# Project-SEA-Stack/HydroChrono

Measured on AMD Instinct MI355X. Metric: hydro-force evals/sec (all bodies), higher is better.
Workload: dtype f64

## Files before the change

hydrochrono_amd/capi.py:

```python
import ctypes as C
import os

_PKG = os.path.dirname(os.path.abspath(__file__))
LIB_PATH = os.path.join(_PKG, "lib", "libhydrochrono_amd.so")
TUNING_LIB_PATH = os.path.join(_PKG, "lib", "libhydrochrono_amd_tuning.so")

HC_OK, HC_ERR_RUNTIME, HC_ERR_OUT_OF_RANGE, HC_ERR_INVALID, HC_ERR_DEVICE, HC_ERR_UNSUPPORTED = range(6)

c_double_p = C.POINTER(C.c_double)
c_int_p = C.POINTER(C.c_int)


class IrregularWaveParams(C.Structure):
    _fields_ = [("num_bodies", C.c_int), ("simulation_dt", C.c_double), ("simulation_duration", C.c_double),
                ("ramp_duration", C.c_double), ("wave_height", C.c_double), ("wave_period", C.c_double),
                ("frequency_min", C.c_double), ("frequency_max", C.c_double), ("nfrequencies", C.c_double),
                ("peak_enhancement_factor", C.c_double), ("is_normalized", C.c_int), ("seed", C.c_int)]


class TaperedDirectOptions(C.Structure):
    _fields_ = [("smoothing", C.c_int), ("window_length", C.c_int), ("rirf_end_time", C.c_double),
                ("taper_start_percent", C.c_double), ("taper_end_percent", C.c_double),
                ("taper_final_amplitude", C.c_double), ("export_plot_csv", C.c_int)]

# ... 12 lines not shown


class MorisonMember(C.Structure):
    _fields_ = [("r0", C.c_double * 3), ("r1", C.c_double * 3), ("d0", C.c_double), ("d1", C.c_double), ("cd", C.c_double),
                ("cm", C.c_double), ("n_seg", C.c_int)]


class SurfacePanel(C.Structure):
    _fields_ = [("c", C.c_double * 3), ("s", C.c_double * 3)]


class RadiationMode(C.Structure):
    _fields_ = [("row", C.c_int), ("col", C.c_int), ("lambda_re", C.c_double), ("lambda_im", C.c_double),
                ("rho_re", C.c_double), ("rho_im", C.c_double)]


class ProfileStats(C.Structure):
    _fields_ = [("hydrostatics_seconds", C.c_double), ("radiation_seconds", C.c_double), ("waves_seconds", C.c_double),
                ("hydrostatics_calls", C.c_int), ("radiation_calls", C.c_int), ("waves_calls", C.c_int),
                ("conv_kernel_seconds", C.c_double), ("conv_kernel_launches", C.c_longlong),
                ("conv_kernel_bytes", C.c_double), ("block_kernel_seconds", C.c_double),
                ("block_kernel_launches", C.c_longlong), ("block_kernel_bytes", C.c_double),
                ("block_kernel_bytes_once", C.c_double),
                ("step_kernel_seconds", C.c_double), ("step_kernel_launches", C.c_longlong),
                ("scatter_kernel_seconds", C.c_double), ("scatter_kernel_launches", C.c_longlong),
                ("direct_dispatches", C.c_longlong), ("hip_launches", C.c_longlong), ("history_rewinds", C.c_longlong),
                ("mini_pass_seconds", C.c_double), ("mini_pass_launches", C.c_longlong), ("queue_parkings", C.c_longlong),
                ("ahead_pass_slices", C.c_longlong), ("ahead_blocks", C.c_longlong),
                ("pass_lane_launches", C.c_longlong),
                ("multi_doorbell_offset_last", C.c_double), ("multi_doorbell_offset_sum", C.c_double), ("multi_calls", C.c_longlong),
                ("slot_state_steps", C.c_longlong), ("wide_fused_steps", C.c_longlong),
                ("schedule_blocks_ahead", C.c_longlong), ("schedule_blocks_at_start", C.c_longlong), ("ring_grows_for_pass", C.c_longlong),
                ("hot_steps", C.c_longlong), ("tail_launches", C.c_longlong), ("tail_seconds", C.c_double),
                ("tail_bytes", C.c_double), ("tail_blocks", C.c_longlong)]


class InitStats(C.Structure):
    _fields_ = [("h5_read_seconds", C.c_double), ("h5_read_bytes", C.c_double), ("rirf_h2d_seconds", C.c_double), ("rirf_h2d_bytes", C.c_double),
                ("rirf_relayout_seconds", C.c_double), ("rirf_relayout_bytes", C.c_double), ("finalize_seconds", C.c_double),
                ("direct_setup_seconds", C.c_double), ("wave_resample_seconds", C.c_double), ("wave_spectrum_seconds", C.c_double),
                ("wave_eta_seconds", C.c_double), ("wave_eta_samples", C.c_longlong), ("wave_eta_components", C.c_longlong),
                ("wave_eta_mode", C.c_int), ("pad_", C.c_int), ("wave_upload_seconds", C.c_double), ("wave_upload_bytes", C.c_double),
                ("wave_total_seconds", C.c_double), ("taper_seconds", C.c_double), ("taper_bytes", C.c_double),
                ("synth_seconds", C.c_double), ("synth_bytes", C.c_double)]


SIGNATURES = {
    "hc_version": (C.c_char_p, []),
    "hc_device_count": (C.c_int, []),
    "hc_device_local_cpus": (C.c_int, [C.c_int, C.c_char_p, C.c_size_t]),
    "hc_bind_thread_to_device": (C.c_int, [C.c_int]),
    "hc_create": (C.c_int, [C.c_int, C.c_int, C.POINTER(C.c_void_p)]),
    "hc_create_sharded": (C.c_int, [C.c_int, C.c_int, C.c_int, C.c_int, C.POINTER(C.c_void_p)]),
    "hc_destroy": (None, [C.c_void_p]),
    "hc_last_error": (C.c_char_p, [C.c_void_p]),
    "hc_set_simulation_parameters": (C.c_int, [C.c_void_p, C.c_double, C.c_double, C.c_double]),
    "hc_set_body_properties": (C.c_int, [C.c_void_p, C.c_int, C.c_double, c_double_p, c_double_p]),
    "hc_set_hydrostatic_stiffness": (C.c_int, [C.c_void_p, C.c_int, c_double_p]),
    "hc_set_added_mass_inf": (C.c_int, [C.c_void_p, C.c_int, c_double_p]),
    "hc_set_rirf": (C.c_int, [C.c_void_p, C.c_int, c_double_p, C.c_int, c_double_p]),
    "hc_set_excitation_rao": (C.c_int, [C.c_void_p, C.c_int, c_double_p, C.c_int, c_double_p, c_double_p]),
    "hc_set_excitation_irf": (C.c_int, [C.c_void_p, C.c_int, c_double_p, C.c_int, c_double_p]),
    "hc_load_bemio_h5": (C.c_int, [C.c_void_p, C.c_char_p]),
    "hc_finalize": (C.c_int, [C.c_void_p]),
    "hc_set_gravity": (C.c_int, [C.c_void_p, c_double_p]),
    "hc_set_wave_none": (C.c_int, [C.c_void_p, C.c_int]),
    "hc_set_wave_regular": (C.c_int, [C.c_void_p, C.c_int, C.c_double, C.c_double]),
# ... 212 lines not shown
```

hydrochrono_amd/csrc/hc_context.hpp:

```cpp
#pragma once
#include <hip/hip_runtime.h>

#include <chrono>
#include <cmath>
#include <deque>
#include <stdexcept>
#include <string>
#include <vector>

#include "../../include/hydrochrono_amd.h"
#include "hc_direct.hpp"
#include "hc_kernels.hpp"
#include "hc_plan.hpp"

namespace hc {

struct Error : std::runtime_error {
    int status;
    Error(int st, const std::string& what) : std::runtime_error(what), status(st) {}
};

#define HC_HIP(expr)                                                                                          \
    do {                                                                                                      \
        hipError_t _e = (expr);                                                                               \
// ... 205 lines not shown
    int first_body = 0, off = 0, L = 0;
    double tau_front = 0.0, tau_back = 0.0;
};

enum WaveKind { kWaveNone = 0, kWaveRegular = 1, kWaveIrregular = 2, kWaveSpectral = 3 };

enum EventKind { kEvConvPlain = 0, kEvPass = 1, kEvStep = 2, kEvScatter = 3, kEvConvExc = 4, kEvMiniPass = 5, kEvTail = 6 };
struct EventPair {
    hipEvent_t a = nullptr, b = nullptr;
    int kind = 0;
    double waves_share = 0.0;
};

}

struct hc_ctx {
    int N = 0, b0 = 0, b1 = 0, nloc = 0, D = 0, Dloc = 0, device = 0;
    hipStream_t stream = nullptr;
    hipStream_t stream_am = nullptr;
    hipEvent_t ev_fin = nullptr, ev_bg = nullptr;
    bool bg_pending = false;
    hipStream_t last_stream = nullptr;
    bool have_last_stream   = false;
    hc::DirectQueue* dq = nullptr;
    bool direct_ready   = false;
    std::string direct_why;
    std::string direct_how = "direct AQL dispatch";
    int path            = 0;
    hc::DirectKernel dk_finalize_slot;
    hc::DirectKernel dk_step_hot[2];
    bool step_hot = false;
    int step_halves = 1;
    bool slot_state = false;
    hc::DirectKernel dk_finalize, dk_scatter, dk_reduce, dk_block16, dk_block32, dk_block64, dk_mini16, dk_mini32, dk_narrow, dk_wide, dk_added_mass, dk_step, dk_near;
    hc::StepTail tail;
    int pending_step  = 0;
    double pending_t  = 0.0;
    int pending_am    = 0;
    bool lost         = false;
    int arm_mode = 1;
    bool arm_after_step = false, arm_after_am = false;
    std::chrono::steady_clock::time_point t_step_end{}, t_am_end{};
    bool have_t_step_end = false, have_t_am_end = false;
    int busy_caller_steps   = 0;
    std::string err;

    bool have_sim = false;
    double rho = 0, g = 0, depth = 0;
    double gsys[3] = {0.0, 0.0, -9.81};
    std::vector<hc::BodyHost> bodies;

    int S = 0;
    std::vector<double> tau, width;
    hc::DeviceBuffer<double> dK, dKproc, d_tau, d_width, d_stage;
    int ntiles = 0, Dpad = 0, ngp = 0, mt = 1, ngroups = 0;
    int conv_mode = 0;
    bool proc_ready = false;
    hc_tapered_direct_options taper{};
    std::string diagnostics_dir;
    bool finalized = false;

    std::deque<double> times;
    std::deque<double> retired;
    int head = -1, Hcap = 0, HcapT = 0;
    hc::DeviceBuffer<double> d_ring_t, d_ring_v, d_ring_vT;
    long long rewinds = 0;
    bool have_prev = false, have_prev_device = false;
// ... 146 lines not shown
```

hydrochrono_amd/csrc/hc_internal.hpp:

```cpp
#pragma once
#include <dlfcn.h>
#include <fcntl.h>
#include <unistd.h>
#include <xmmintrin.h>

#include <algorithm>
#include <chrono>
#include <cmath>
#include <cstdint>
#include <cstdio>
#include <cstdlib>
#include <cstring>
#include <fstream>
#include <limits>
#include <memory>
#include <string>
#include <vector>

#include "hc_context.hpp"
#include "hc_history.hpp"
#include "hc_host_math.hpp"

namespace hc {
void eta_synthesis_fft(const std::vector<double>& t, const std::vector<double>& amp, const std::vector<double>& omega,
// ... 112 lines not shown
    return RaoBracket{k0, k0 + 1, idx_des - std::floor(idx_des)};
}
inline void rao_bracket_check(const RaoBracket& br, int nw) {
    if (br.k0 < 0 || br.k0 + 1 >= nw) throw Error(HC_ERR_OUT_OF_RANGE, "regular wave frequency outside the BEM frequency list");
}
void apply_wave_directions(hc_ctx* c, const std::vector<double>& theta, bool commit, bool force);

struct StepFlags {
    bool hs = true, rad = true, waves = true;
    bool scratch_out = false;
};
struct HostState {
    const double *pos, *rpy, *linvel, *angvel;
    double canary;
};
void enqueue_step(hc_ctx* c, double t, const double* d_state, double* d_user_out, hipStream_t stream, StepFlags f,
                  unsigned long long* host_tagged = nullptr, unsigned long long seq = 0, bool defer_tail = false, const HostState* host_state = nullptr);
void enqueue_tail(hc_ctx* c);

bool wave_window_ok(const hc_ctx* c, double t);
int live_samples(const hc_ctx* c, double t_query);
double* rows_P(hc_ctx* c, bool next);
double* rows_E(hc_ctx* c, bool next);

struct StepViews {
    hc::Panel kex;
    hc::EtaTable ex;
};
StepViews make_views(const hc_ctx* c);
struct PassSetup {
    hc::BlockArgs b;
    bool exc_block = false;
    double rad_once = 0.0, exc_once = 0.0, bytes_steps = 0.0;
};
PassSetup make_pass(hc_ctx* c, bool with_exc, bool next_block, int head_lags = 0);
void issue_pass_chunks(hc_ctx* c, const PassSetup& ps, int first, int last, bool with_items, hipStream_t stream, bool direct, int lane = 0);
struct TailRows {
    const double* tail[hc::kTailLevelsMax] = {nullptr, nullptr, nullptr};
    int j0[hc::kTailLevelsMax]             = {0, 0, 0};
};
void issue_pass_reduce(hc_ctx* c, const PassSetup& ps, double* P, double* E, hipStream_t stream, bool direct, int lane = 0, const TailRows* tail = nullptr);
void launch_pass(hc_ctx* c, hipStream_t stream, bool with_exc, bool direct = false, bool spec_goes_on = false);
void spec_drop(hc_ctx* c, bool k_changed);
void spec_build_khat(hc_ctx* c, hc_ctx::SpectralLevel& lev);
void launch_mini_pass(hc_ctx* c, int i0, hipStream_t stream, bool direct, int next_kw = 0, int lane = 0);
void ahead_drop(hc_ctx* c);
void ahead_issue_slice(hc_ctx* c, hipStream_t stream, bool direct);
void ahead_begin(hc_ctx* c, hipStream_t stream, bool with_exc, bool direct);
bool ahead_expected(const hc_ctx* c, unsigned long long ended_serial);
bool ahead_adoptable(const hc_ctx* c, unsigned long long ended_serial);
bool pass_lane_ready(hc_ctx* c);
void pass_lane_drain(hc_ctx* c);

}
}
```

hydrochrono_amd/csrc/hc_kernels.hip:

```cpp
#include "hc_kernels.hpp"

#include <algorithm>
#include <cstdint>
#include <cstdlib>

namespace hc {

static constexpr int kConvThreads = 256;
static constexpr int kWave        = 64;

typedef double dvec2 __attribute__((ext_vector_type(2)));
typedef double dvec2u __attribute__((ext_vector_type(2), aligned(8)));
typedef double dvec4 __attribute__((ext_vector_type(4)));

__host__ __device__ inline size_t panel_offset(int ngp, int row, int f) {
    const int rt = row >> 4, ri = row & 15, gp = f >> 3, j = (f >> 2) & 1, kk = f & 3;
    return ((static_cast<size_t>(rt) * ngp + gp) * 64 + (kk * 16 + ri)) * 2 + j;
}

__global__ void __launch_bounds__(256) relayout_rirf_kernel(const double* __restrict__ Kb, double* __restrict__ K, int ngp, int D, int S,
                                                             int row0, double scale) {
    const size_t F   = (size_t)S * D;
    const size_t gid = (size_t)blockIdx.x * blockDim.x + threadIdx.x;
    if (gid >= 6 * F) return;
// ... 716 lines not shown
                ++s_c;
            } while (cb_c >= D);
            load_weights();
        }
    };

    const int nfrag = (gp1 - gp0 - wave + 3) / 4;
#pragma unroll
    for (int r = 0; r < R; ++r) issue(r);
    for (int i = 0; i < nfrag; i += R) {
#pragma unroll
        for (int r = 0; r < R; ++r) {
            consume(r);
            issue(r);
        }
    }

#pragma unroll
    for (int tb = 0; tb < NB; ++tb) {
        __syncthreads();
#pragma unroll
        for (int m = 0; m < MT; ++m)
#pragma unroll
            for (int r = 0; r < 4; ++r) red[((size_t)wave * MT + m) * 256 + (kk + 4 * r) * 16 + jstep] = acc[tb][m][r];
        __syncthreads();
        for (int idx = tid; idx < MT * 256; idx += kConvThreads) {
            const int m = idx >> 8, el = idx & 255, row = el >> 4, j = el & 15;
            const double v = ((red[(0 * MT + m) * 256 + el] + red[(1 * MT + m) * 256 + el]) + red[(2 * MT + m) * 256 + el]) + red[(3 * MT + m) * 256 + el];
            a.partials[((size_t)chunk * L + 16 * tb + j) * a.Dpad + (grp * MT + m) * 16 + row] = v;
        }
    }
}

template <int MT, int R, int NB, int WPS = (NB == 1 ? 2 : 1)>
__global__ void __launch_bounds__(kConvThreads, WPS) conv_block_kernel(BlockArgs a) {
    extern __shared__ __align__(16) unsigned char smem_raw[];
    double* front = reinterpret_cast<double*>(smem_raw);
    const int nt  = a.max_steps_per_chunk * 16 * NB;
    double* t_wo  = front + a.lds_front_doubles;
    double* t_wn  = t_wo + nt;
    int* t_oo     = reinterpret_cast<int*>(t_wn + nt);
    int* t_on     = t_oo + nt;

    const int r     = (int)blockIdx.x % (8 * a.ngroups);
    const int chunk = a.chunk_first + ((int)blockIdx.x / (8 * a.ngroups)) * 8 + (r & 7);
    const int grp   = r >> 3;
    if (chunk >= (a.chunk_last > 0 ? a.chunk_last : a.nchunks)) return;

    if constexpr (NB > 2) {
        block_rad_stream_uni<MT, R, NB>(a, chunk, grp, front, t_wo, t_wn, t_oo, t_on);
    } else {
        if ((a.hist.D & 7) == 0 && (size_t)a.hist.D * a.hist.HcapT < ((size_t)1 << 28)) block_rad_stream_uni<MT, R, NB>(a, chunk, grp, front, t_wo, t_wn, t_oo, t_on);
        else block_rad_stream<MT, (NB > 1) ? 2 : R, NB, false>(a, chunk, grp, front, t_wo, t_wn, t_oo, t_on);
    }
    const int RG      = a.ngroups;
    const int n_items = a.nchunks_ex * NB * RG;
    if (n_items > 0) {
        __shared__ int s_item;
        for (;;) {
            __syncthreads();
            if (threadIdx.x == 0) s_item = atomicAdd(a.item_counter, 1);
            __syncthreads();
            const int it = s_item;
            if (it >= n_items) break;
            const int e = it / (NB * RG), rem = it - e * (NB * RG), tb = rem / RG, rg = rem - tb * RG;
            block_exc_work<MT>(a, rg, e, 16 * tb, front);
        }
    }
}

template <class KernelT>
static void allow_dynamic_lds(KernelT kernel, size_t smem, size_t& granted) {
    if (smem > 64 * 1024 && smem > granted) {
        (void)hipFuncSetAttribute(reinterpret_cast<const void*>(kernel), hipFuncAttributeMaxDynamicSharedMemorySize, (int)smem);
        granted = smem;
    }
}

template <int MT, int R>
static void launch_conv_block_mt(const BlockArgs& b, int nblocks, size_t smem, hipStream_t stream) {
    static size_t granted16 = 0, granted32 = 0;
    if (b.depth == 32) {
        allow_dynamic_lds(conv_block_kernel<MT, R + 1, 2>, smem, granted32);
        hipLaunchKernelGGL((conv_block_kernel<MT, R + 1, 2>), dim3(nblocks), dim3(kConvThreads), smem, stream, b);
    } else {
        allow_dynamic_lds(conv_block_kernel<MT, R, 1>, smem, granted16);
        hipLaunchKernelGGL((conv_block_kernel<MT, R, 1>), dim3(nblocks), dim3(kConvThreads), smem, stream, b);
    }
}

#ifdef HC_TUNING
static void launch_conv_block64(const BlockArgs& b, int nblocks, size_t smem, hipStream_t stream) {
    static size_t granted = 0;
    allow_dynamic_lds(conv_block_kernel<kBlock64MT, 4, 4, 1>, smem, granted);
    hipLaunchKernelGGL((conv_block_kernel<kBlock64MT, 4, 4, 1>), dim3(nblocks), dim3(kConvThreads), smem, stream, b);
}
#endif

BlockLaunch block_launch_config(const BlockArgs& a, int mt, BlockArgs* b) {
    BlockLaunch l;
    const int nlaunch = (a.chunk_last > 0 ? a.chunk_last : a.nchunks) - a.chunk_first;
// ... 1 lines not shown
    *b        = a;
    b->lds_front_doubles = max(4 * kUWave, 4 * mt * 256);
    l.smem    = (size_t)b->lds_front_doubles * sizeof(double) + (size_t)max(1, a.max_steps_per_chunk) * b->depth * 24;
#ifdef HC_TUNING
    if (a.depth == 64) {
        l.MT  = kBlock64MT;
        l.NB  = 4;
        l.R   = 4;
        l.WPS = 1;
        return l;
    }
#endif
    l.MT  = (mt == 6 || mt == 4 || mt == 2) ? mt : 1;
    const int R16 = l.MT == 6 ? 3 : 4;
    l.NB  = a.depth == 32 ? 2 : 1;
    l.R   = a.depth == 32 ? R16 + 1 : R16;
    l.WPS = l.NB == 1 ? 2 : 1;
    return l;
}

void launch_conv_block(const BlockArgs& a, int mt, hipStream_t stream) {
    BlockArgs b;
    const BlockLaunch l = block_launch_config(a, mt, &b);
    const int nblocks   = l.nblocks;
    const size_t smem   = l.smem;
    if (nblocks <= 0) return;
#ifdef HC_TUNING
    if (b.depth == 64) { launch_conv_block64(b, nblocks, smem, stream); return; }
#endif
    if (mt == 6) launch_conv_block_mt<6, 3>(b, nblocks, smem, stream);
    else if (mt == 4) launch_conv_block_mt<4, 4>(b, nblocks, smem, stream);
    else if (mt == 2) launch_conv_block_mt<2, 4>(b, nblocks, smem, stream);
    else launch_conv_block_mt<1, 4>(b, nblocks, smem, stream);
}

__device__ __forceinline__ double lane16_sum(double v) {
#pragma unroll
    for (int off = 8; off >= 1; off >>= 1) v += __shfl_xor(v, off, 16);
    return v;
}

__global__ void __launch_bounds__(256) reduce_block_kernel(ReduceArgs a) {
    if (blockIdx.x == 0 && threadIdx.x == 0) *a.item_counter = 0;
    const double* __restrict__ partials = a.partials;
    const int sub = threadIdx.x & 15;
    const int n   = a.depth * a.Dpad;
    int out       = blockIdx.x * 16 + (threadIdx.x >> 4);
    const bool exc = out >= n;
    if (exc) out -= n;
    const int first = exc ? a.nchunks_rad : a.rad_first, count = exc ? a.nchunks_ex : a.nchunks_rad - a.rad_first;
    const int o     = out < n ? out : 0;
    double v = 0.0;
    if (a.narrow) {
        const int j = o / a.Dpad, row = o - j * a.Dpad;
        for (int c = sub; c < count; c += 8 * 16) {
            double w[8];
#pragma unroll
            for (int k = 0; k < 8; ++k) {
                const int cc = first + c + 16 * k;
                const int jj = (c + 16 * k) < count ? j - (int)a.jbase[cc] : -1;
                w[k]         = (jj >= 0 && jj < 16) ? partials[((size_t)cc * 16 + jj) * a.Dpad + row] : 0.0;
            }
#pragma unroll
            for (int k = 0; k < 8; ++k) v += w[k];
        }
    } else {
// ... 1227 lines not shown
```

hydrochrono_amd/csrc/hc_kernels.hpp:

```cpp
#pragma once
#include <hip/hip_runtime.h>

#include <cstddef>

#include "hc_limits.hpp"
#include "hc_tail.hpp"

namespace hc {


struct Panel {
    const double* base;
    int ntiles;
    int ngp;
};
inline size_t panel_doubles(int ntiles, int ngp) { return static_cast<size_t>(ntiles) * ngp * 128; }

struct HistoryView {
    const double* state;
    int N, D;
    double t;
    const double* ring_t;
    const double* ring_v;
    const double* ring_vT;
// ... 227 lines not shown
    int grid = 0, threads = 256;
    size_t smem = 0;
};
struct NearLaunch {
    int grid = 0;
    size_t smem = 0;
};
int near_slices_for(int D);
NearLaunch near_launch_config(NearArgs& a);
struct WideLaunch {
    int grid = 0;
    size_t smem = 0;
};
WideLaunch wide_launch_config(WideStepArgs& a);
struct ScatterLaunch {
    int grid = 0;
    size_t smem = 0;
};
ScatterLaunch scatter_launch_config(ScatterArgs& a);
FinalizeLaunch finalize_launch_config(FinalizeArgs& a);
struct StepLaunch {
    int nblocks = 0;
    size_t smem = 0;
    int MT = 0;
    static constexpr int U = 2;
};
StepLaunch step_launch_config(const StepArgs& a, int mt);
struct BlockLaunch {
    int nblocks = 0;
    size_t smem = 0;
    int MT = 0, R = 0, NB = 0, WPS = 0;
};
BlockLaunch block_launch_config(const BlockArgs& a, int mt, BlockArgs* with_lds_layout);

void launch_relayout_rirf(const double* d_Kb_6xDxS, double* d_K, int ngp, int D, int S, int row0, double scale, hipStream_t stream);
void launch_relayout_rowmajor(const double* d_src, int rows, int cols, double* d_panel, int ngp, int row0, hipStream_t stream);
void launch_conv_step(const StepArgs& a, int mt, hipStream_t stream);
void launch_conv_block(const BlockArgs& a, int mt, hipStream_t stream);
void launch_reduce_block(const ReduceArgs& r, hipStream_t stream);
int reduce_block_grid(const ReduceArgs& r);
void launch_finalize(const FinalizeArgs& a, hipStream_t stream);
void launch_near_split(const NearArgs& a, hipStream_t stream);
void launch_wide_step(const WideStepArgs& a, hipStream_t stream);
void launch_scatter(const ScatterArgs& a, hipStream_t stream);
void launch_taper(const TaperArgs& a, hipStream_t stream);
void launch_eta_synthesis(const double* d_t, int nt, const double* d_amp, const double* d_omega, const double* d_phase, int nf,
                          double ramp_duration, double* d_eta, hipStream_t stream);
void launch_added_mass_mv(const double* d_M, int rows, int cols, const double* d_w, double c, double* d_R, hipStream_t stream);
void launch_added_mass_mv_tagged(const double* d_M, int rows, int cols, const double* d_w, const double* d_R_in, double c,
                                 unsigned long long* d_tagged, unsigned long long seq, const double* d_canary_in, unsigned long long* d_canary_out,
                                 hipStream_t stream);
void launch_unrelayout(const Panel& K, int Dloc, int D, int S, double* d_out, hipStream_t stream);
void launch_extract_series(const Panel& K, int row, int col, int D, int S, double* d_out, hipStream_t stream);
void launch_ring_transpose(const double* d_ring_v, int Hcap, int HcapT, int D, double* d_ring_vT, hipStream_t stream);
void launch_synth_rirf(double* d_K, int ntiles, int ngp, int Dloc, int D, int S, int row0, double dt, unsigned long long seed, double rho,
                       hipStream_t stream);

struct TailKhatArgs {
    Panel K;
    const double* width;
    const double* tw;
    double* Khat;
    int Dloc, D, S, NP;
};

struct TailFwdArgs {
    const double* ring_vT;
    int HcapT, Hcap, head;
    int D, S, NP;
    const double* tw;
    double* Xw;
// ... 30 lines not shown
```

hydrochrono_amd/csrc/hc_pass.cpp:

```cpp
#include "hc_internal.hpp"

using namespace hc::detail;

namespace hc {
namespace detail {

StepViews make_views(const hc_ctx* c) {
    StepViews v{};
    const bool irregular = c->wave_kind == hc::kWaveIrregular;
    v.kex.base   = c->d_kex.p;
    v.kex.ntiles = c->ntiles;
    v.kex.ngp    = c->ngp_ex;
    v.ex.L        = c->L;
    v.ex.ex_tau   = c->d_ex_tau.p;
    v.ex.ex_width = c->d_ex_width.p;
    v.ex.eta_t    = c->d_eta_t.p;
    v.ex.eta      = c->d_eta.p;
    v.ex.nt       = c->nt;
    v.ex.eta_dt   = irregular ? (c->eta_record ? c->eta_h : c->irr.simulation_dt) : 1.0;
    v.ex.eta_t0   = (irregular && !c->eta_t.empty()) ? c->eta_t.front() : 0.0;
    return v;
}


// ... 63 lines not shown
    b.ngroups     = c->ntiles / (L == 64 ? hc::kBlock64MT : c->mt_block);
    double samples = 0.0;
    for (int j = 0; j < L; ++j) samples += std::max(0, b.F / c->D - b.s_cut[j]);
    const double rad_16 = 8.0 * samples * (static_cast<double>(c->Dloc) * c->D + c->D);
    const double exc_16 = exc_block ? 8.0 * L * (static_cast<double>(c->Dloc) * c->L + c->L) : 0.0;
    ps.bytes_steps = rad_16 + exc_16;
    ps.rad_once    = 8.0 * (static_cast<double>(c->Dloc) * b.F + b.F);
    ps.exc_once    = exc_block ? 8.0 * (static_cast<double>(c->Dloc) * c->L + c->L) : 0.0;
    if (HC_TUNE_INT("HC_DEBUG_PLAN", 0) != 0) {
        std::fprintf(stderr, "[hc] pass%s t0=%.6f dt=%.17g Hv=%d F/D=%d nchunks=%d exc=%d\n     s_cut:", next_block ? " (next block)" : "", pl.tgrid[0], pl.dt, Hv,
                     b.F / c->D, b.nchunks, (int)exc_block);
        for (int j = 0; j < L; ++j) std::fprintf(stderr, " %d", b.s_cut[j]);
        std::fprintf(stderr, "\n     s_defer:");
        for (int j = 0; j < L; ++j) std::fprintf(stderr, " %d", b.s_defer[j]);
        std::fprintf(stderr, "\n     scat:");
        for (int i = 1; i <= L; ++i) std::fprintf(stderr, " [%d,%d]", pl.scat_lo[i], pl.scat_hi[i]);
        std::fprintf(stderr, "\n");
    }
    return ps;
}

void issue_pass_chunks(hc_ctx* c, const PassSetup& ps, int first, int last, bool with_items, hipStream_t stream, bool direct, int lane) {
    hc::BlockArgs b = ps.b;
    b.chunk_first   = first;
    b.chunk_last    = last;
    if (!with_items) b.nchunks_ex = 0;
    const double share_rad = static_cast<double>(last - first) / std::max(1, ps.b.nchunks);
    const double rad_once = ps.rad_once * share_rad, exc_once = with_items ? ps.exc_once : 0.0;
    c->prof.block_kernel_bytes      = ps.bytes_steps * (rad_once + exc_once) / std::max(1.0, ps.rad_once + ps.exc_once);
    c->prof.block_kernel_bytes_once = rad_once + exc_once;
    const double exc_share = exc_once / std::max(1.0, rad_once + exc_once);
    const int L  = c->lookahead;
    const int mt = L == 64 ? hc::kBlock64MT : c->mt_block;
    if (direct) {
        hc::BlockArgs b2;
        const hc::BlockLaunch l = hc::block_launch_config(b, mt, &b2);
        if (l.nblocks <= 0) return;
        c->dq->dispatch(L == 64 ? c->dk_block64 : (L == 32 ? c->dk_block32 : c->dk_block16), static_cast<uint32_t>(l.nblocks), 256, static_cast<uint32_t>(l.smem), &b2, sizeof b2,
                        direct_tag(c, hc::kEvPass), exc_share, lane);
        c->prof.direct_dispatches += 1;
        if (lane == 2) c->prof.pass_lane_launches += 1;
        return;
    }
    hc::EventPair* ev = ev_begin(c, hc::kEvPass, stream, exc_share);
    hc::launch_conv_block(b, mt, stream);
    ev_end(ev, stream);
    c->prof.hip_launches += 1;
}

void issue_pass_reduce(hc_ctx* c, const PassSetup& ps, double* P, double* E, hipStream_t stream, bool direct, int lane, const TailRows* tail) {
    const hc::BlockArgs& b = ps.b;
    hc::ReduceArgs r{b.partials, b.nchunks, b.nchunks_ex, c->Dpad, c->lookahead, P, E, b.item_counter, 0, 0, 0, 0};
    if (tail) {
        r.tail      = tail->tail[0];
        r.tail_j0   = tail->j0[0];
        r.tail_b    = tail->tail[1];
        r.tail_b_j0 = tail->j0[1];
        r.tail_c    = tail->tail[2];
        r.tail_c_j0 = tail->j0[2];
    }
    if (direct) {
        c->dq->dispatch(c->dk_reduce, static_cast<uint32_t>(hc::reduce_block_grid(r)), 256, 0, &r, sizeof r, -1, 0.0, lane);
        c->prof.direct_dispatches += 1;
        return;
    }
    hc::launch_reduce_block(r, stream);
    c->prof.hip_launches += 1;
}

void spec_drop(hc_ctx* c, bool k_changed) {
    c->spec.active = false;
    c->spec.far_cur = c->spec.far_next = 0;
    if (k_changed)
        for (auto& f : c->spec_form) f.khat_ok = false;
}

namespace {

// ... 142 lines not shown
        if (b.n >= n) return false;
        fresh.push_back(&b);
        b.alloc(n);
        return true;
    };
    try {
        for (int l = 0; l < nlev; ++l) {
            auto& lev = form.lev[l];
            lev.lv = lv[l];
            const size_t bins = static_cast<size_t>(lv[l].bins), ncols = static_cast<size_t>(lv[l].NP) * c->D;
            grow(lev.xw, 2 * bins * ncols);
            grow(lev.y, 4 * bins * c->Dloc);
            if (grow(lev.out, static_cast<size_t>(lv[l].P) * c->Dpad)) {
                HC_HIP(hipMemsetAsync(lev.out.p, 0, lev.out.n * sizeof(double), c->stream));
                HC_HIP(hipStreamSynchronize(c->stream));
            }
            if (grow(lev.khat, 2 * bins * c->Dloc * ncols)) form.khat_ok = false;
        }
    } catch (const Error&) {
        (void)hipGetLastError();
        for (auto* b : fresh) b->release();
        form.khat_ok      = false;
        c->radiation_tail = 0;
        return false;
    }
    for (int l = 0; l < nlev; ++l) spec_twiddles(c, form.lev[l]);
    if (!form.khat_ok) {
        for (int l = 0; l < nlev; ++l) spec_build_khat(c, form.lev[l]);
        form.khat_ok = true;
    }
    return form.khat_ok;
}

}

void launch_pass(hc_ctx* c, hipStream_t stream, bool with_exc, bool direct, bool spec_goes_on) {
    auto& sp = c->spec;
    const auto& pl = c->plan;
    const int L = c->lookahead;
    const int fi = spec_form_index(c);
    bool use_tail = false;
    if (spec_goes_on && sp.active && sp.form == fi && sp.k < sp.Q && std::fabs(pl.dt - sp.dt) <= 1e-9 * sp.dt) {
        const double tol = std::max(1e-9 * pl.dt, 64.0 * std::numeric_limits<double>::epsilon() * std::fabs(pl.tgrid[1]));
        use_tail = std::fabs(pl.tgrid[1] - (sp.t0 + sp.k * L * sp.dt)) <= tol;
    }
    if (!use_tail) {
        const bool follows = spec_goes_on && sp.active && sp.form == fi && sp.k == sp.Q &&
                             std::fabs(pl.tgrid[1] - (sp.t0 + sp.k * L * sp.dt)) <=
                                 std::max(1e-9 * pl.dt, 64.0 * std::numeric_limits<double>::epsilon() * std::fabs(pl.tgrid[1])) &&
                             std::fabs(pl.dt - sp.dt) <= 1e-9 * sp.dt;
        const unsigned far_made = follows ? sp.far_next : 0u;
        sp.active = false;
        if (spec_eligible(c, direct) && spec_ready(c)) {
            sp.form     = fi;
            sp.cur      = follows ? 1 - sp.cur : sp.cur;
            sp.far_cur  = far_made;
            sp.far_next = 0;
            sp.Q        = hc::tail_level_blocks(c->spec_form[fi].lev[0].lv, L);
            sp.k        = 0;
            sp.t0       = pl.tgrid[1];
            sp.dt       = pl.dt;
            sp.active   = true;
            use_tail = true;
        }
    }
    if (!use_tail) {
        const PassSetup ps = make_pass(c, with_exc, false);
        c->plan.has_exc    = ps.exc_block;
        issue_pass_chunks(c, ps, 0, ps.b.nchunks, true, stream, direct);
        issue_pass_reduce(c, ps, rows_P(c, false), rows_E(c, false), stream, direct);
        return;
    }
    auto& form = c->spec_form[fi];
    const int j0 = sp.k * L;
    TailRows rows;
    for (int l = 0; l < form.nlev; ++l) {
        auto& lev = form.lev[l];
        if (hc::tail_level_starts(lev.lv, j0)) spec_level_start(c, lev, l == 0, stream, direct);
        rows.tail[l] = lev.out.p;
        rows.j0[l]   = j0 % lev.lv.period;
    }
    const PassSetup ps = make_pass(c, with_exc, false, hc::tail_head_lags(&form.lev[form.nlev - 1].lv, 1));
    c->plan.has_exc    = ps.exc_block;
    issue_pass_chunks(c, ps, 0, ps.b.nchunks, true, stream, direct);
    issue_pass_reduce(c, ps, rows_P(c, false), rows_E(c, false), stream, direct, 0, &rows);
    const auto& top = form.lev[0];
    const int NP = top.lv.NP;
    if (hc::tail_level_far_ahead(top.lv) && sp.k >= 1) {
        const int ch = sp.k - 1, nch = hc::tail_far_chunks(sp.Q);
        int lo, hi;
        hc::tail_level_chunk_bins(top.lv, ch, nch, &lo, &hi);
        spec_dispatch_gemv(c, top, stream, direct, lo, hi, c->D, NP * c->D, hc::tail_x_shift(true, c->D), nullptr,
                           top.y.p + static_cast<size_t>(1 - sp.cur) * 2 * top.lv.bins * c->Dloc);
        sp.far_next |= 1u << ch;
    }
    sp.k += 1;
    sp.serial = c->plan_serial;
    c->prof.tail_blocks += 1;
}

void ahead_drop(hc_ctx* c) { c->ahead.active = false; }

void reset_schedule_state(hc_ctx* c) {
    c->gap_seen = c->gap_long = c->gap_long_lo = 0;
    c->gap_hint  = -1.0;
    c->ahead_now = hc::near_slices_for(c->D) > 1 && c->gap_threshold <= 0.0;
}

bool schedule_ahead_for_next_block(hc_ctx* c) {
    if (c->pass_ahead == 0 || c->lookahead > 32) return false;
    if (c->pass_ahead == 1) return true;
    if (!pass_ahead_size_ok(c)) return false;
    if (c->gap_seen >= std::max(4, c->lookahead / 4)) {
        c->ahead_now = 2 * (c->ahead_now ? c->gap_long_lo : c->gap_long) > c->gap_seen;
        c->gap_seen = c->gap_long = c->gap_long_lo = 0;
    }
// ... 230 lines not shown
```

hydrochrono_amd/csrc/hc_runtime.cpp:

```cpp
#include "hc_internal.hpp"

#include <sched.h>

#include <cctype>

#include <atomic>

using namespace hc::detail;

template <class T>
void hc::BarBuffer<T>::alloc(size_t count) {
    if (p) (void)hipFree(p);
    p       = nullptr;
    n       = 0;
    host_ok = false;
    if (count == 0) return;
    static const bool disabled = HC_TUNE_INT("HC_NO_BAR_STATE", 0) != 0;
    if (disabled) return;
    void* q = nullptr;
    if (hipExtMallocWithFlags(&q, count * sizeof(T), hipDeviceMallocFinegrained) != hipSuccess) {
        (void)hipGetLastError();
        return;
    }
    p = static_cast<T*>(q);
// ... 605 lines not shown
    c->dk_tail_gemv = q->find("tail_gemvENS_12TailGemvArgsE");
    bool tail_ok    = c->dk_tail_gemv.kernarg == sizeof(hc::TailGemvArgs) && !c->dk_tail_gemv.priv;
    for (int i = 0; i < 3; ++i) {
        char frag[64];
        std::snprintf(frag, sizeof frag, "tail_fft_fwdILi%dEEEvNS_11TailFwdArgsE", 256 << i);
        c->dk_tail_fwd[i] = q->find(frag);
        std::snprintf(frag, sizeof frag, "tail_fft_invILi%dEEEvNS_11TailInvArgsE", 256 << i);
        c->dk_tail_inv[i] = q->find(frag);
        tail_ok = tail_ok && c->dk_tail_fwd[i].kernarg == sizeof(hc::TailFwdArgs) && c->dk_tail_inv[i].kernarg == sizeof(hc::TailInvArgs) && !c->dk_tail_fwd[i].priv &&
                  !c->dk_tail_inv[i].priv;
    }
    if (!tail_ok) {
        c->dk_tail_gemv = hc::DirectKernel{};
        for (int i = 0; i < 3; ++i) c->dk_tail_fwd[i] = c->dk_tail_inv[i] = hc::DirectKernel{};
    }
    c->dk_added_mass = q->find("added_mass_mv_tagged_kernelE");
    {
        hc::StepArgs a{};
        a.ngroups = 1;
        const hc::StepLaunch l = hc::step_launch_config(a, c->mt);
        char frag[64];
        std::snprintf(frag, sizeof frag, "conv_step_kernelILi%dELi%dEEEv", l.MT, hc::StepLaunch::U);
        c->dk_step = q->find(frag);
        if (c->dk_step.kernarg != sizeof(hc::StepArgs) || c->dk_step.priv != 0) c->dk_step = hc::DirectKernel{};
    }
    for (int depth : {16, 32}) {
        hc::BlockArgs a{}, b{};
        a.depth = depth;
        a.ngroups = 1;
        const hc::BlockLaunch l = hc::block_launch_config(a, c->mt_block, &b);
        char frag[96];
        std::snprintf(frag, sizeof frag, "conv_block_kernelILi%dELi%dELi%dELi%dEEEv", l.MT, l.R, l.NB, l.WPS);
        (depth == 16 ? c->dk_block16 : c->dk_block32) = q->find(frag);
        const hc::BlockLaunch lm = hc::block_launch_config(a, c->mt_mini, &b);
        std::snprintf(frag, sizeof frag, "conv_block_kernelILi%dELi%dELi%dELi%dEEEv", lm.MT, lm.R, lm.NB, lm.WPS);
        (depth == 16 ? c->dk_mini16 : c->dk_mini32) = q->find(frag);
        if (depth == 16) {
            const hc::BlockLaunch ln = hc::block_launch_config(a, c->mt_narrow, &b);
            std::snprintf(frag, sizeof frag, "conv_block_kernelILi%dELi%dELi%dELi%dEEEv", ln.MT, ln.R, ln.NB, ln.WPS);
            c->dk_narrow = q->find(frag);
        }
    }
#ifdef HC_TUNING
    {
        hc::BlockArgs a{}, b{};
        a.depth   = 64;
        a.ngroups = 1;
        const hc::BlockLaunch l = hc::block_launch_config(a, hc::kBlock64MT, &b);
        char frag[96];
        std::snprintf(frag, sizeof frag, "conv_block_kernelILi%dELi%dELi%dELi%dEEEv", l.MT, l.R, l.NB, l.WPS);
        c->dk_block64 = q->find(frag);
        if (c->dk_block64.kernarg != sizeof(hc::BlockArgs) || c->dk_block64.priv != 0) c->dk_block64 = hc::DirectKernel{};
    }
#endif
    if (!c->dk_narrow.ok() || c->dk_narrow.priv || c->dk_narrow.kernarg != sizeof(hc::BlockArgs)) {
        c->direct_why = "the narrow short-pass variant of the pass kernel is missing from hc_kernels.co";
        return;
    }
    if (!c->dk_mini16.ok() || !c->dk_mini32.ok() || c->dk_mini16.priv || c->dk_mini32.priv || c->dk_mini16.kernarg != sizeof(hc::BlockArgs) ||
        c->dk_mini32.kernarg != sizeof(hc::BlockArgs)) {
        c->direct_why = "the short-pass variant of the pass kernel is missing from hc_kernels.co";
        return;
    }
    if (!c->dk_finalize.ok() || !c->dk_scatter.ok() || !c->dk_reduce.ok() || !c->dk_block16.ok() || !c->dk_block32.ok() || !c->dk_near.ok()) {
        c->direct_why = "a kernel of this configuration is missing from hc_kernels.co";
        return;
// ... 59 lines not shown
```

include/hydrochrono_amd.h:

```cpp
#ifndef HYDROCHRONO_AMD_H
#define HYDROCHRONO_AMD_H

#include <stddef.h>

#ifdef __cplusplus
extern "C" {
#endif

typedef struct hc_ctx hc_ctx;

typedef enum hc_status {
    HC_OK               = 0,
    HC_ERR_RUNTIME      = 1,
    HC_ERR_OUT_OF_RANGE = 2,
    HC_ERR_INVALID      = 3,
    HC_ERR_DEVICE       = 4,
    HC_ERR_UNSUPPORTED  = 5
} hc_status;

const char* hc_version(void);
int hc_device_count(void);
int hc_device_local_cpus(int device_id, char* out, size_t out_bytes);
int hc_bind_thread_to_device(int device_id);
int hc_create(int num_bodies, int device_id, hc_ctx** out);
// ... 100 lines not shown
typedef struct hc_profile_stats {
    double hydrostatics_seconds, radiation_seconds, waves_seconds;
    int hydrostatics_calls, radiation_calls, waves_calls;
    double conv_kernel_seconds;
    long long conv_kernel_launches;
    double conv_kernel_bytes;
    double block_kernel_seconds;
    long long block_kernel_launches;
    double block_kernel_bytes;
    double block_kernel_bytes_once;
    double step_kernel_seconds;
    long long step_kernel_launches;
    double scatter_kernel_seconds;
    long long scatter_kernel_launches;
    long long direct_dispatches, hip_launches;
    long long history_rewinds;
    double mini_pass_seconds;
    long long mini_pass_launches;
    long long queue_parkings;
    long long ahead_pass_slices;
    long long ahead_blocks;
    long long pass_lane_launches;
    double multi_doorbell_offset_last, multi_doorbell_offset_sum;
    long long multi_calls;
    long long slot_state_steps;
    long long wide_fused_steps;
    long long schedule_blocks_ahead, schedule_blocks_at_start;
    long long ring_grows_for_pass;
    long long hot_steps;
    long long tail_launches;
    double tail_seconds;
    double tail_bytes;
    long long tail_blocks;
} hc_profile_stats;
int hc_enable_profiling(hc_ctx* ctx, int on);
int hc_get_profile(hc_ctx* ctx, hc_profile_stats* out);
int hc_reset_profile(hc_ctx* ctx);

typedef struct hc_init_stats {
    double h5_read_seconds, h5_read_bytes;
    double rirf_h2d_seconds, rirf_h2d_bytes;
    double rirf_relayout_seconds, rirf_relayout_bytes;
    double finalize_seconds;
    double direct_setup_seconds;
    double wave_resample_seconds;
    double wave_spectrum_seconds;
    double wave_eta_seconds;
    long long wave_eta_samples, wave_eta_components;
    int wave_eta_mode, pad_;
    double wave_upload_seconds, wave_upload_bytes;
    double wave_total_seconds;
    double taper_seconds, taper_bytes;
    double synth_seconds, synth_bytes;
} hc_init_stats;
int hc_get_init_stats(const hc_ctx* ctx, hc_init_stats* out);

int hc_get_sizes(hc_ctx* ctx, int* N, int* n_local, int* S, int* L, int* nf, int* nt, int* H, int* Hcap);
int hc_get_rirf_width(hc_ctx* ctx, double* w_S);
int hc_get_rirf_effective(hc_ctx* ctx, double* out_DlocalxDxS);
int hc_get_rirf_value(hc_ctx* ctx, int row_local, int col, int st, double* out);
int hc_get_excitation_irf_resampled(hc_ctx* ctx, int body, double* t_L, double* width_L, double* vals_6xL);
int hc_get_excitation_irf_size(hc_ctx* ctx, int body, int* L);
int hc_get_spectrum(hc_ctx* ctx, double* f, double* S, double* df, double* phase, double* k);
int hc_get_eta_table(hc_ctx* ctx, double* t_nt, double* eta_nt);
int hc_export_irregular_inputs_h5(hc_ctx* ctx, const char* path);
int hc_get_regular_coeffs(hc_ctx* ctx, double* mag_D, double* phase_D, double* wavenumber);
// ... 128 lines not shown
```

Measured before the change: 85530.

## Add specialised head-pass block kernel for uniform-grid radiation convolution

Adds a head_block_kernel that streams the radiation convolution for the head pass with per-step offsets computed in registers, instead of building per-step weight/offset tables in LDS as conv_block_kernel does. The new kernel uses only the front LDS region, which lowers shared-memory use and table setup, and is chosen at pass time when the plan is uniform, has no deferred or mini-window lags and the history fits. It adds new dispatch selection, kernel lookup and a profiling counter, and risks mismatched behaviour if the eligibility checks miss a case.

```diff
diff --git a/hydrochrono_amd/capi.py b/hydrochrono_amd/capi.py
--- a/hydrochrono_amd/capi.py
+++ b/hydrochrono_amd/capi.py
@@ -68,7 +68,7 @@
                 ("slot_state_steps", C.c_longlong), ("wide_fused_steps", C.c_longlong),
                 ("schedule_blocks_ahead", C.c_longlong), ("schedule_blocks_at_start", C.c_longlong), ("ring_grows_for_pass", C.c_longlong),
                 ("hot_steps", C.c_longlong), ("tail_launches", C.c_longlong), ("tail_seconds", C.c_double),
-                ("tail_bytes", C.c_double), ("tail_blocks", C.c_longlong)]
+                ("tail_bytes", C.c_double), ("tail_blocks", C.c_longlong), ("head_kernel_launches", C.c_longlong)]
 
 
 class InitStats(C.Structure):
diff --git a/hydrochrono_amd/csrc/hc_context.hpp b/hydrochrono_amd/csrc/hc_context.hpp
--- a/hydrochrono_amd/csrc/hc_context.hpp
+++ b/hydrochrono_amd/csrc/hc_context.hpp
@@ -261,7 +261,7 @@
     bool step_hot = false;
     int step_halves = 1;
     bool slot_state = false;
-    hc::DirectKernel dk_finalize, dk_scatter, dk_reduce, dk_block16, dk_block32, dk_block64, dk_mini16, dk_mini32, dk_narrow, dk_wide, dk_added_mass, dk_step, dk_near;
+    hc::DirectKernel dk_finalize, dk_scatter, dk_reduce, dk_block16, dk_block32, dk_block64, dk_head16, dk_head32, dk_mini16, dk_mini32, dk_narrow, dk_wide, dk_added_mass, dk_step, dk_near;
     hc::StepTail tail;
     int pending_step  = 0;
     double pending_t  = 0.0;
diff --git a/hydrochrono_amd/csrc/hc_internal.hpp b/hydrochrono_amd/csrc/hc_internal.hpp
--- a/hydrochrono_amd/csrc/hc_internal.hpp
+++ b/hydrochrono_amd/csrc/hc_internal.hpp
@@ -168,6 +168,7 @@
     hc::BlockArgs b;
     bool exc_block = false;
     double rad_once = 0.0, exc_once = 0.0, bytes_steps = 0.0;
+    bool head_kernel = false;
 };
 PassSetup make_pass(hc_ctx* c, bool with_exc, bool next_block, int head_lags = 0);
 void issue_pass_chunks(hc_ctx* c, const PassSetup& ps, int first, int last, bool with_items, hipStream_t stream, bool direct, int lane = 0);
diff --git a/hydrochrono_amd/csrc/hc_kernels.hip b/hydrochrono_amd/csrc/hc_kernels.hip
--- a/hydrochrono_amd/csrc/hc_kernels.hip
+++ b/hydrochrono_amd/csrc/hc_kernels.hip
@@ -772,27 +772,146 @@
     }
 }
 
-template <int MT, int R, int NB, int WPS = (NB == 1 ? 2 : 1)>
-__global__ void __launch_bounds__(kConvThreads, WPS) conv_block_kernel(BlockArgs a) {
-    extern __shared__ __align__(16) unsigned char smem_raw[];
-    double* front = reinterpret_cast<double*>(smem_raw);
-    const int nt  = a.max_steps_per_chunk * 16 * NB;
-    double* t_wo  = front + a.lds_front_doubles;
-    double* t_wn  = t_wo + nt;
-    int* t_oo     = reinterpret_cast<int*>(t_wn + nt);
-    int* t_on     = t_oo + nt;
-
-    const int r     = (int)blockIdx.x % (8 * a.ngroups);
-    const int chunk = a.chunk_first + ((int)blockIdx.x / (8 * a.ngroups)) * 8 + (r & 7);
-    const int grp   = r >> 3;
-    if (chunk >= (a.chunk_last > 0 ? a.chunk_last : a.nchunks)) return;
-
-    if constexpr (NB > 2) {
-        block_rad_stream_uni<MT, R, NB>(a, chunk, grp, front, t_wo, t_wn, t_oo, t_on);
-    } else {
-        if ((a.hist.D & 7) == 0 && (size_t)a.hist.D * a.hist.HcapT < ((size_t)1 << 28)) block_rad_stream_uni<MT, R, NB>(a, chunk, grp, front, t_wo, t_wn, t_oo, t_on);
-        else block_rad_stream<MT, (NB > 1) ? 2 : R, NB, false>(a, chunk, grp, front, t_wo, t_wn, t_oo, t_on);
-    }
+template <int MT, int R, int NB>
+__device__ __forceinline__ void head_rad_stream(const BlockArgs& a, const int chunk, const int grp, double* red) {
+    static_assert(NB <= 2, "head pass: depth 16 or 32");
+    constexpr int L = 16 * NB;
+    const int tid = threadIdx.x, lane = tid & 63;
+    const int wave = __builtin_amdgcn_readfirstlane(tid >> 6);
+    const int kk = lane >> 4, jstep = lane & 15;
+    const int D = a.hist.D;
+    const int gp0 = chunk * a.chunk_gp;
+    const int gp1 = min((a.F + 7) >> 3, gp0 + a.chunk_gp);
+    const int s_last = a.F / D - 1;
+    const int Hcap   = a.hist.Hcap;
+
+    int s_from[NB], hj[NB];
+#pragma unroll
+    for (int tb = 0; tb < NB; ++tb) {
+        const int j = 16 * tb + jstep;
+        s_from[tb]  = max(a.s_cut[j], j + 1);
+        hj[tb]      = a.hist.head + j;
+    }
+
+    dvec4 acc[NB][MT];
+#pragma unroll
+    for (int tb = 0; tb < NB; ++tb)
+#pragma unroll
+        for (int m = 0; m < MT; ++m) acc[tb][m] = dvec4{0.0, 0.0, 0.0, 0.0};
+    const char* __restrict__ kb    = reinterpret_cast<const char*>(a.K.base) + ((size_t)(grp * MT) * a.K.ngp) * 1024;
+    const size_t tile_bytes        = (size_t)a.K.ngp * 1024;
+    const unsigned lane16          = (unsigned)lane * 16u;
+    const char* __restrict__ ringb = reinterpret_cast<const char*>(a.hist.ring_vT);
+    const unsigned col_bytes       = (unsigned)a.hist.HcapT * 8u;
+
+    dvec2 kv[R][MT];
+    double v[R][2][NB];
+
+    int gp_i = gp0 + wave;
+    int s_i = (gp_i * 8) / D, cb_i = gp_i * 8 - s_i * D;
+    unsigned cby = (unsigned)(cb_i + kk) * col_bytes;
+    unsigned boo[NB];
+    auto set_offsets = [&]() {
+        const int s = min(s_i, s_last);
+#pragma unroll
+        for (int tb = 0; tb < NB; ++tb) {
+            int x = hj[tb] - s;
+            x += (x < 0) ? Hcap : 0;
+            x -= (x >= Hcap) ? Hcap : 0;
+            boo[tb] = (s >= s_from[tb]) ? (unsigned)x * 8u : 0u;
+        }
+    };
+    set_offsets();
+    auto issue = [&](const int slot) {
+        const int gpc = min(gp_i, gp1 - 1);
+        const char* __restrict__ kg = kb + (size_t)gpc * 1024;
+#pragma unroll
+        for (int m = 0; m < MT; ++m) kv[slot][m] = __builtin_nontemporal_load(reinterpret_cast<const dvec2*>(kg + m * tile_bytes + lane16));
+#pragma unroll
+        for (int h = 0; h < 2; ++h)
+#pragma unroll
+            for (int tb = 0; tb < NB; ++tb) {
+                const unsigned cb = cby + (unsigned)(4 * h) * col_bytes;
+                v[slot][h][tb]    = *reinterpret_cast<const double*>(ringb + (cb + boo[tb]));
+            }
+        gp_i += 4;
+        cb_i += 32;
+        cby += 32u * col_bytes;
+        if (cb_i >= D) {
+            do {
+                cb_i -= D;
+                cby -= (unsigned)D * col_bytes;
+                ++s_i;
+            } while (cb_i >= D);
+            set_offsets();
+        }
+    };
+
+    int gp_c = gp0 + wave;
+    int s_c = (gp_c * 8) / D, cb_c = gp_c * 8 - s_c * D;
+    double cw[NB];
+    auto set_weights = [&]() {
+        const double w = a.width[min(s_c, s_last)];
+#pragma unroll
+        for (int tb = 0; tb < NB; ++tb) cw[tb] = (s_c >= s_from[tb]) ? w : 0.0;
+    };
+    set_weights();
+    auto consume = [&](const int slot) {
+        if (gp_c < gp1) {
+            double u[2][NB];
+#pragma unroll
+            for (int h = 0; h < 2; ++h)
+#pragma unroll
+                for (int tb = 0; tb < NB; ++tb) u[h][tb] = cw[tb] * v[slot][h][tb];
+#pragma unroll
+            for (int tb = 0; tb < NB; ++tb)
+#pragma unroll
+                for (int m = 0; m < MT; ++m) acc[tb][m] = __builtin_amdgcn_mfma_f64_16x16x4f64(kv[slot][m].x, u[0][tb], acc[tb][m], 0, 0, 0);
+#pragma unroll
+            for (int tb = 0; tb < NB; ++tb)
+#pragma unroll
+                for (int m = 0; m < MT; ++m) acc[tb][m] = __builtin_amdgcn_mfma_f64_16x16x4f64(kv[slot][m].y, u[1][tb], acc[tb][m], 0, 0, 0);
+        }
+        gp_c += 4;
+        cb_c += 32;
+        if (cb_c >= D) {
+            do {
+                cb_c -= D;
+                ++s_c;
+            } while (cb_c >= D);
+            set_weights();
+        }
+    };
+
+    const int nfrag = (gp1 - gp0 - wave + 3) / 4;
+#pragma unroll
+    for (int r = 0; r < R; ++r) issue(r);
+    for (int i = 0; i < nfrag; i += R) {
+#pragma unroll
+        for (int r = 0; r < R; ++r) {
+            consume(r);
+            issue(r);
+        }
+    }
+
+#pragma unroll
+    for (int tb = 0; tb < NB; ++tb) {
+        __syncthreads();
+#pragma unroll
+        for (int m = 0; m < MT; ++m)
+#pragma unroll
+            for (int r = 0; r < 4; ++r) red[((size_t)wave * MT + m) * 256 + (kk + 4 * r) * 16 + jstep] = acc[tb][m][r];
+        __syncthreads();
+        for (int idx = tid; idx < MT * 256; idx += kConvThreads) {
+            const int m = idx >> 8, el = idx & 255, row = el >> 4, j = el & 15;
+            const double s = ((red[(0 * MT + m) * 256 + el] + red[(1 * MT + m) * 256 + el]) + red[(2 * MT + m) * 256 + el]) + red[(3 * MT + m) * 256 + el];
+            a.partials[((size_t)chunk * L + 16 * tb + j) * a.Dpad + (grp * MT + m) * 16 + row] = s;
+        }
+    }
+}
+
+template <int MT, int NB>
+__device__ __forceinline__ void block_exc_items(const BlockArgs& a, double* front) {
     const int RG      = a.ngroups;
     const int n_items = a.nchunks_ex * NB * RG;
     if (n_items > 0) {
@@ -807,6 +926,43 @@
             block_exc_work<MT>(a, rg, e, 16 * tb, front);
         }
     }
+}
+
+template <int MT, int R, int NB, int WPS = (NB == 1 ? 2 : 1)>
+__global__ void __launch_bounds__(kConvThreads, WPS) head_block_kernel(BlockArgs a) {
+    extern __shared__ __align__(16) unsigned char smem_raw[];
+    double* front = reinterpret_cast<double*>(smem_raw);
+    touch_args<sizeof(BlockArgs)>();
+    const int r     = (int)blockIdx.x % (8 * a.ngroups);
+    const int chunk = a.chunk_first + ((int)blockIdx.x / (8 * a.ngroups)) * 8 + (r & 7);
+    const int grp   = r >> 3;
+    if (chunk >= (a.chunk_last > 0 ? a.chunk_last : a.nchunks)) return;
+    head_rad_stream<MT, R, NB>(a, chunk, grp, front);
+    block_exc_items<MT, NB>(a, front);
+}
+
+template <int MT, int R, int NB, int WPS = (NB == 1 ? 2 : 1)>
+__global__ void __launch_bounds__(kConvThreads, WPS) conv_block_kernel(BlockArgs a) {
+    extern __shared__ __align__(16) unsigned char smem_raw[];
+    double* front = reinterpret_cast<double*>(smem_raw);
+    const int nt  = a.max_steps_per_chunk * 16 * NB;
+    double* t_wo  = front + a.lds_front_doubles;
+    double* t_wn  = t_wo + nt;
+    int* t_oo     = reinterpret_cast<int*>(t_wn + nt);
+    int* t_on     = t_oo + nt;
+
+    const int r     = (int)blockIdx.x % (8 * a.ngroups);
+    const int chunk = a.chunk_first + ((int)blockIdx.x / (8 * a.ngroups)) * 8 + (r & 7);
+    const int grp   = r >> 3;
+    if (chunk >= (a.chunk_last > 0 ? a.chunk_last : a.nchunks)) return;
+
+    if constexpr (NB > 2) {
+        block_rad_stream_uni<MT, R, NB>(a, chunk, grp, front, t_wo, t_wn, t_oo, t_on);
+    } else {
+        if ((a.hist.D & 7) == 0 && (size_t)a.hist.D * a.hist.HcapT < ((size_t)1 << 28)) block_rad_stream_uni<MT, R, NB>(a, chunk, grp, front, t_wo, t_wn, t_oo, t_on);
+        else block_rad_stream<MT, (NB > 1) ? 2 : R, NB, false>(a, chunk, grp, front, t_wo, t_wn, t_oo, t_on);
+    }
+    block_exc_items<MT, NB>(a, front);
 }
 
 template <class KernelT>
@@ -874,6 +1030,33 @@
     else if (mt == 4) launch_conv_block_mt<4, 4>(b, nblocks, smem, stream);
     else if (mt == 2) launch_conv_block_mt<2, 4>(b, nblocks, smem, stream);
     else launch_conv_block_mt<1, 4>(b, nblocks, smem, stream);
+}
+
+BlockLaunch head_launch_config(const BlockArgs& a, int mt, BlockArgs* b) {
+    BlockLaunch l = block_launch_config(a, mt, b);
+    l.smem        = (size_t)b->lds_front_doubles * sizeof(double);
+    return l;
+}
+
+bool head_kernel_fits(const BlockArgs& a) {
+    return (a.depth == 16 || a.depth == 32) && (a.hist.D & 7) == 0 && (size_t)a.hist.D * a.hist.HcapT < ((size_t)1 << 28) && a.F > 0 &&
+           a.hist.Hcap > a.F / a.hist.D + a.depth;
+}
+
+template <int MT, int R>
+static void launch_head_block_mt(const BlockArgs& b, int nblocks, size_t smem, hipStream_t stream) {
+    if (b.depth == 32) hipLaunchKernelGGL((head_block_kernel<MT, R + 1, 2>), dim3(nblocks), dim3(kConvThreads), smem, stream, b);
+    else hipLaunchKernelGGL((head_block_kernel<MT, R, 1>), dim3(nblocks), dim3(kConvThreads), smem, stream, b);
+}
+
+void launch_head_block(const BlockArgs& a, int mt, hipStream_t stream) {
+    BlockArgs b;
+    const BlockLaunch l = head_launch_config(a, mt, &b);
+    if (l.nblocks <= 0) return;
+    if (mt == 6) launch_head_block_mt<6, 3>(b, l.nblocks, l.smem, stream);
+    else if (mt == 4) launch_head_block_mt<4, 4>(b, l.nblocks, l.smem, stream);
+    else if (mt == 2) launch_head_block_mt<2, 4>(b, l.nblocks, l.smem, stream);
+    else launch_head_block_mt<1, 4>(b, l.nblocks, l.smem, stream);
 }
 
 __device__ __forceinline__ double lane16_sum(double v) {
diff --git a/hydrochrono_amd/csrc/hc_kernels.hpp b/hydrochrono_amd/csrc/hc_kernels.hpp
--- a/hydrochrono_amd/csrc/hc_kernels.hpp
+++ b/hydrochrono_amd/csrc/hc_kernels.hpp
@@ -283,11 +283,14 @@
     int MT = 0, R = 0, NB = 0, WPS = 0;
 };
 BlockLaunch block_launch_config(const BlockArgs& a, int mt, BlockArgs* with_lds_layout);
+BlockLaunch head_launch_config(const BlockArgs& a, int mt, BlockArgs* with_lds_layout);
+bool head_kernel_fits(const BlockArgs& a);
 
 void launch_relayout_rirf(const double* d_Kb_6xDxS, double* d_K, int ngp, int D, int S, int row0, double scale, hipStream_t stream);
 void launch_relayout_rowmajor(const double* d_src, int rows, int cols, double* d_panel, int ngp, int row0, hipStream_t stream);
 void launch_conv_step(const StepArgs& a, int mt, hipStream_t stream);
 void launch_conv_block(const BlockArgs& a, int mt, hipStream_t stream);
+void launch_head_block(const BlockArgs& a, int mt, hipStream_t stream);
 void launch_reduce_block(const ReduceArgs& r, hipStream_t stream);
 int reduce_block_grid(const ReduceArgs& r);
 void launch_finalize(const FinalizeArgs& a, hipStream_t stream);
diff --git a/hydrochrono_amd/csrc/hc_pass.cpp b/hydrochrono_amd/csrc/hc_pass.cpp
--- a/hydrochrono_amd/csrc/hc_pass.cpp
+++ b/hydrochrono_amd/csrc/hc_pass.cpp
@@ -119,18 +119,21 @@
     const double exc_share = exc_once / std::max(1.0, rad_once + exc_once);
     const int L  = c->lookahead;
     const int mt = L == 64 ? hc::kBlock64MT : c->mt_block;
+    const bool head = ps.head_kernel && L != 64;
+    if (head) c->prof.head_kernel_launches += 1;
     if (direct) {
         hc::BlockArgs b2;
-        const hc::BlockLaunch l = hc::block_launch_config(b, mt, &b2);
+        const hc::BlockLaunch l = head ? hc::head_launch_config(b, mt, &b2) : hc::block_launch_config(b, mt, &b2);
         if (l.nblocks <= 0) return;
-        c->dq->dispatch(L == 64 ? c->dk_block64 : (L == 32 ? c->dk_block32 : c->dk_block16), static_cast<uint32_t>(l.nblocks), 256, static_cast<uint32_t>(l.smem), &b2, sizeof b2,
-                        direct_tag(c, hc::kEvPass), exc_share, lane);
+        const hc::DirectKernel& dk = head ? (L == 32 ? c->dk_head32 : c->dk_head16) : (L == 64 ? c->dk_block64 : (L == 32 ? c->dk_block32 : c->dk_block16));
+        c->dq->dispatch(dk, static_cast<uint32_t>(l.nblocks), 256, static_cast<uint32_t>(l.smem), &b2, sizeof b2, direct_tag(c, hc::kEvPass), exc_share, lane);
         c->prof.direct_dispatches += 1;
         if (lane == 2) c->prof.pass_lane_launches += 1;
         return;
     }
     hc::EventPair* ev = ev_begin(c, hc::kEvPass, stream, exc_share);
-    hc::launch_conv_block(b, mt, stream);
+    if (head) hc::launch_head_block(b, mt, stream);
+    else hc::launch_conv_block(b, mt, stream);
     ev_end(ev, stream);
     c->prof.hip_launches += 1;
 }
@@ -339,6 +342,22 @@
     return form.khat_ok;
 }
 
+bool head_kernel_ok(const hc_ctx* c, const hc::BlockArgs& b, int head_lags, bool direct) {
+    const bool enabled = HC_TUNE_INT("HC_HEAD_KERNEL", 1) != 0;
+    const auto& pl = c->plan;
+    const int L    = c->lookahead;
+    if (!enabled || (L != 16 && L != 32) || !hc::head_kernel_fits(b)) return false;
+    if (direct && !(L == 32 ? c->dk_head32 : c->dk_head16).ok()) return false;
+    if (!pl.valid || pl.own_zero || pl.sub != 0 || b.mini_kw != 0) return false;
+    for (int j = 0; j < L; ++j)
+        if (b.s_defer[j] >= 0 || b.s_cut[j] >= head_lags) return false;
+#ifdef HC_TUNING
+    if (!hc::tail_grid_ok(c->times, c->tau, pl.dt, pl.tgrid[1]))
+        throw Error(HC_ERR_RUNTIME, "head pass of a tail block: the history has left the uniform grid inside a top period");
+#endif
+    return true;
+}
+
 }
 
 void launch_pass(hc_ctx* c, hipStream_t stream, bool with_exc, bool direct, bool spec_goes_on) {
@@ -387,8 +406,10 @@
         rows.tail[l] = lev.out.p;
         rows.j0[l]   = j0 % lev.lv.period;
     }
-    const PassSetup ps = make_pass(c, with_exc, false, hc::tail_head_lags(&form.lev[form.nlev - 1].lv, 1));
-    c->plan.has_exc    = ps.exc_block;
+    const int head_lags = hc::tail_head_lags(&form.lev[form.nlev - 1].lv, 1);
+    PassSetup ps        = make_pass(c, with_exc, false, head_lags);
+    c->plan.has_exc     = ps.exc_block;
+    ps.head_kernel      = head_kernel_ok(c, ps.b, head_lags, direct);
     issue_pass_chunks(c, ps, 0, ps.b.nchunks, true, stream, direct);
     issue_pass_reduce(c, ps, rows_P(c, false), rows_E(c, false), stream, direct, 0, &rows);
     const auto& top = form.lev[0];
diff --git a/hydrochrono_amd/csrc/hc_runtime.cpp b/hydrochrono_amd/csrc/hc_runtime.cpp
--- a/hydrochrono_amd/csrc/hc_runtime.cpp
+++ b/hydrochrono_amd/csrc/hc_runtime.cpp
@@ -661,6 +661,10 @@
         char frag[96];
         std::snprintf(frag, sizeof frag, "conv_block_kernelILi%dELi%dELi%dELi%dEEEv", l.MT, l.R, l.NB, l.WPS);
         (depth == 16 ? c->dk_block16 : c->dk_block32) = q->find(frag);
+        std::snprintf(frag, sizeof frag, "head_block_kernelILi%dELi%dELi%dELi%dEEEv", l.MT, l.R, l.NB, l.WPS);
+        hc::DirectKernel& dh = depth == 16 ? c->dk_head16 : c->dk_head32;
+        dh = q->find(frag);
+        if (dh.kernarg != sizeof(hc::BlockArgs) || dh.priv != 0) dh = hc::DirectKernel{};
         const hc::BlockLaunch lm = hc::block_launch_config(a, c->mt_mini, &b);
         std::snprintf(frag, sizeof frag, "conv_block_kernelILi%dELi%dELi%dELi%dEEEv", lm.MT, lm.R, lm.NB, lm.WPS);
         (depth == 16 ? c->dk_mini16 : c->dk_mini32) = q->find(frag);
diff --git a/include/hydrochrono_amd.h b/include/hydrochrono_amd.h
--- a/include/hydrochrono_amd.h
+++ b/include/hydrochrono_amd.h
@@ -156,6 +156,7 @@
     double tail_seconds;
     double tail_bytes;
     long long tail_blocks;
+    long long head_kernel_launches;
 } hc_profile_stats;
 int hc_enable_profiling(hc_ctx* ctx, int on);
 int hc_get_profile(hc_ctx* ctx, hc_profile_stats* out);
```

New measurement: 81010. 5.3% lower.
